# cmavro/GNN-RAG

Measured on AMD Instinct MI355X. Metric: kg_edges_aggregated_per_sec, higher is better.
Workload: dtype f32

## Files before the change

gnn-rag_amd/csrc/dense_internal.h:

```cpp
#pragma once
#include "gnnrag_common.h"

namespace gnnrag {

int tables_vq_launch_z(const gnnrag_csr* csr, const void* planes, const float* ins, const float* W, float* P, int32_t D,
                       int32_t I, int32_t only_dir, float* zero, int64_t zero_n, hipStream_t stream);

int tables_vq_lite_launch_z(const gnnrag_csr* csr, const void* planes, const float* ins, const float* W, float* P, int32_t D,
                            int32_t I, int32_t only_dir, float* zero, int64_t zero_n, hipStream_t stream);

int update_b3_launch_z(const float* h, const float* nbr, const float* W, const float* b, const float* w_s,
                       const float* b_s, const float* mask, float* h_out, float* score, int64_t BN, int32_t D,
                       int32_t ldw, hipStream_t stream, bool score_zeroed);

int update_score_fused_rows(const float* h, const float* nbr, const uint8_t* add_flag, const float* W, const float* b,
                            const float* w_s, const float* b_s, const float* mask, float* h_out, float* score,
                            int64_t BN, int32_t D, int32_t I, int32_t math, hipStream_t stream, bool score_zeroed);
int update_b3_launch_f(const float* h, const float* nbr, const uint8_t* add_flag, const float* W, const float* b,
                       const float* w_s, const float* b_s, const float* mask, float* h_out, float* score, int64_t BN,
                       int32_t D, int32_t ldw, hipStream_t stream, bool score_zeroed);

bool update_rows_supported(const float* h, const float* nbr, const float* W, const float* h_out, int64_t BN, int32_t D,
                           int32_t I, int32_t math);
bool update_b3_shape_ok(int64_t BN, int32_t D, int32_t ldw);
int tables_small_launch(const gnnrag_csr* csr, const float* T_fwd, const float* T_inv, const float* ins, const float* W,
                        float* P, int32_t D, int32_t I, hipStream_t stream);

int frontier_build_z(const gnnrag_csr* csr, const float* dist, void* fws, size_t fws_bytes, float* zero_a,
                     int64_t zero_na, float* zero_b, int64_t zero_nb, hipStream_t stream);
const uint8_t* frontier_row_flags(const gnnrag_csr* csr, const void* fws);

int update_score_fused_z(const float* h, const float* nbr, const float* W, const float* b, const float* w_s,
                         const float* b_s, const float* mask, float* h_out, float* score, int64_t BN, int32_t D,
                         int32_t I, int32_t math, hipStream_t stream, bool score_zeroed);

bool rel_transform_accepts(const float* relfeat_fwd, const float* relfeat_inv, int64_t R1, int32_t D, int32_t L,
                           const gnnrag_layer_params* layers, int32_t pos_rows, const float* T_out, const void* planes_out);

}
```

gnn-rag_amd/csrc/softmax_layer.hip:

```cpp
#include "gnnrag_common.h"
#include "dense_internal.h"

#include <map>
#include <vector>

#ifndef GNNRAG_OVERLAP_TABLES_DEFAULT
#define GNNRAG_OVERLAP_TABLES_DEFAULT 0
#endif
#ifndef GNNRAG_OVERLAP_PROJ_DEFAULT
#define GNNRAG_OVERLAP_PROJ_DEFAULT 0
#endif

namespace gnnrag {

template <int ITEMS>
__global__ __launch_bounds__(1024) void k_masked_softmax(const float* __restrict__ score,
                                                         float* __restrict__ dist, int N) {
  __shared__ float red[16];
  __shared__ float bcast;
  const float* s = score + (size_t)blockIdx.x * N;
  float* o = dist + (size_t)blockIdx.x * N;
  const int lane = threadIdx.x & 63, wave = threadIdx.x >> 6;
  float v[ITEMS > 0 ? ITEMS : 1];

// ... 291 lines not shown
  path &= 0xf;
  if (path == GNNRAG_PATH_AUTO)
    path = fused_is_cheaper(csr->B, csr->N, csr->rel_total, D, I) ? GNNRAG_PATH_FUSED : GNNRAG_PATH_UNFUSED;
  if (path == GNNRAG_PATH_FUSED) {
    float* P = P_done ? P_done : (float*)(base + w.P);
    float* nbr = (float*)(base + w.nbr);
    const bool one_dir = only >= 0 && gnnrag_aggregate_fused_variant(csr, D) != GNNRAG_WALK_L2_GATHER;
    const bool fr_aligned = ((((uintptr_t)ins | (uintptr_t)W_e2e | (uintptr_t)T_fwd | (uintptr_t)T_inv | (uintptr_t)P |
                               (uintptr_t)nbr | (uintptr_t)dist) & 15) == 0) && csr->N > 0;
    const bool frontier_form = seed_prior && only < 0 && fr_aligned && gnnrag_frontier_supported(csr, D) && csr->rel_total > 0;
    if (t_ready && !frontier_form) GNNRAG_HIP(hipStreamWaitEvent((hipStream_t)stream, t_ready, 0));
    if (frontier_form) {
      void* fws = base + w.fws;
      const bool gated = update_rows_supported(h, nbr, W_e2e, h_out, BN, D, I, math);
      if (!gated) GNNRAG_HIP(hipMemsetAsync(nbr, 0, (size_t)BN * D * sizeof(float), (hipStream_t)stream));
      rc = frontier_build_z(csr, dist, fws, w.fws_bytes, score_out, BN, nbr + (size_t)BN * D, D, (hipStream_t)stream);
      if (t_ready) GNNRAG_HIP(hipStreamWaitEvent((hipStream_t)stream, t_ready, 0));
      if (rc) return rc;
      rc = gnnrag_relation_tables_frontier(csr, fws, T_fwd, T_inv, ins, W_e2e, P, D, I, stream);
      if (rc) return rc;
      rc = gnnrag_aggregate_fused_frontier(csr, fws, dist, P, nbr, D, stream);
      if (rc) return rc;
      rc = update_score_fused_rows(h, nbr, gated ? frontier_row_flags(csr, fws) : nullptr, W_e2e, b_e2e, w_score, b_score,
                                   mask, h_out, score_out, BN, D, I, math, (hipStream_t)stream, true);
      if (rc) return rc;
      return finish_softmax(csr, w, base, score_out, dist_out, D, only < 0, pairs_for_next, stream);
    }
    rc = GNNRAG_E_UNSUPPORTED;
    bool score_zeroed = false;
    if (P_done) {
      rc = 0;
      score_zeroed = true;
    } else if (planes && math != GNNRAG_MATH_FP32 && csr->rel_total > 0) {
      const char* menv = getenv("GNNRAG_TABLES_LITE_MAIN");
      rc = ((menv && menv[0] == '1') ? tables_vq_lite_launch_z : tables_vq_launch_z)(
          csr, planes, ins, W_e2e, P, D, I, one_dir ? only : -1, score_out, BN, (hipStream_t)stream);
      score_zeroed = rc == 0;
    }
    if (rc == GNNRAG_E_UNSUPPORTED) rc = gnnrag_relation_tables(csr, T_fwd, T_inv, ins, W_e2e, P, D, I, math, stream);
    if (rc) return rc;
    rc = aggregate_fused_dirs(csr, dist, P, nbr, D, one_dir ? 2 - only : 0, base + w.partial, w.partial_bytes,
                              (hipStream_t)stream, pairs_ready && !one_dir);
    if (rc) return rc;
    rc = update_score_fused_z(h, nbr, W_e2e, b_e2e, w_score, b_score, mask, h_out, score_out, BN, D, I, math,
                              (hipStream_t)stream, score_zeroed);
    if (rc) return rc;
    return finish_softmax(csr, w, base, score_out, dist_out, D, only < 0, pairs_for_next, stream);
  } else {
    if (t_ready) GNNRAG_HIP(hipStreamWaitEvent((hipStream_t)stream, t_ready, 0));
    float* agg = (float*)(base + w.agg);
    rc = gnnrag_aggregate(csr, dist, ins, T_fwd, T_inv, agg, D, I, base + w.partial, w.partial_bytes, stream);
    if (rc) return rc;
    rc = gnnrag_update_score(h, agg, W_e2e, b_e2e, w_score, b_score, mask, h_out, score_out, BN, D, I, math,
                             stream);
    if (rc) return rc;
  }
  return gnnrag_masked_softmax(score_out, dist_out, csr->B, csr->N, stream);
}

static int rel_projections(const gnnrag_csr* csr, int32_t n, const gnnrag_layer_params* layers,
                           const float* relfeat_fwd, const float* relfeat_inv, int32_t pos_rows, float* T,
                           void* planes, bool* planes_written, int32_t D, int32_t math, gnnrag_stream_t stream) {
  *planes_written = false;
  if ((D & 3) == 0) {
    const int rc = gnnrag_rel_transform(relfeat_fwd, relfeat_inv, csr->R1, D, n, layers, pos_rows, T, planes, stream);
    if (rc == 0) *planes_written = planes != nullptr;
    if (rc != GNNRAG_E_UNSUPPORTED) return rc;
  }
// ... 76 lines not shown
  path &= ~GNNRAG_PATH_REUSE_PROJ;
  if (reuse) {
    planes_written = want_planes && rel_transform_accepts(relfeat_fwd, relfeat_inv, csr->R1, D, L, layers, pos_rows, Tall,
                                                          planes_all);
  } else if (upfront) {
    const char* penv = getenv("GNNRAG_OVERLAP_PROJ");
    const bool proj_side = fused && (path & GNNRAG_PATH_SEED_PRIOR) && (penv ? penv[0] != '0' : GNNRAG_OVERLAP_PROJ_DEFAULT != 0);
    OverlapRes* pr = nullptr;
    if (proj_side) {
      const int rc0 = overlap_res(L, &pr);
      if (rc0) return rc0;
      GNNRAG_HIP(hipEventRecord(pr->fork, (hipStream_t)stream));
      GNNRAG_HIP(hipStreamWaitEvent(pr->side, pr->fork, 0));
    }
    const int rc = rel_projections(csr, L, layers, relfeat_fwd, relfeat_inv, pos_rows, Tall,
                                   want_planes ? planes_all : nullptr, &planes_written, D, math,
                                   proj_side ? (gnnrag_stream_t)pr->side : stream);
    if (proj_side) {
      GNNRAG_HIP(hipEventRecord(pr->done[0], pr->side));
      if (rc) (void)hipStreamWaitEvent((hipStream_t)stream, pr->done[0], 0);
      else t_ready = pr->done[0];
    }
    if (rc) return rc;
  }
  const bool overlap = upfront && want_planes && planes_written && fused && (path & ~0xf & ~GNNRAG_PATH_SEED_PRIOR) == 0 &&
                       overlap_shape_ok(csr, L, D, I) && overlap_enabled() &&
                       ((((uintptr_t)ins | (uintptr_t)planes_all) & 15) == 0);
  OverlapRes* ov = nullptr;
  char* P_extra = planes_all + align_up(tables_vq_shape_ok(D, I) ? (size_t)L * plane_bytes : 0, 256);
  const size_t p_bytes = overlap_p_bytes(csr, D);
  bool side_ok[64] = {false};
  const char* genv = getenv("GNNRAG_OVERLAP_GATE");
  const bool gate = !(genv && genv[0] == '0');
  const char* lenv = getenv("GNNRAG_TABLES_LITE");
  const bool lite = !(lenv && lenv[0] == '0');
  auto side_tables = [&](int j) -> int {
    if (j >= 64 || (((uintptr_t)layers[j].W_e2e) & 15) != 0) return 0;
    const int rc = (lite ? tables_vq_lite_launch_z : tables_vq_launch_z)(
        csr, planes_all + (size_t)j * plane_bytes, ins, layers[j].W_e2e, (float*)(P_extra + (size_t)(j - 1) * p_bytes), D, I, -1,
        score_out + (size_t)j * BN, (int64_t)BN, ov->side);
    if (rc == GNNRAG_E_UNSUPPORTED) return 0;
    if (rc) return rc;
    side_ok[j] = true;
    GNNRAG_HIP(hipEventRecord(ov->done[j], ov->side));
    return 0;
  };
  auto side_join_all = [&](int from) {
    if (!ov) return;
    (void)hipEventRecord(ov->done[0], ov->side);
    (void)hipStreamWaitEvent((hipStream_t)stream, ov->done[0], 0);
    (void)from;
  };
  if (overlap && L <= 64) {
    { const int rc = overlap_res(L, &ov); if (rc) return rc; }
    GNNRAG_HIP(hipEventRecord(ov->fork, (hipStream_t)stream));
    GNNRAG_HIP(hipStreamWaitEvent(ov->side, ov->fork, 0));
    int rc_side = 0;
    for (int j = 1; j < (gate ? 2 : L) && !rc_side; ++j) rc_side = side_tables(j);
    if (rc_side) {
      side_join_all(0);
      return rc_side;
    }
  }
  const float* h = h0;
  const float* dist = dist0;
  bool pairs_ready = false;
  for (int j = 0; j < L; ++j) {
    const gnnrag_layer_params& p = layers[j];
    float* hj = h_out + (size_t)j * BN * D;
    float* sj = score_out + (size_t)j * BN;
    float* dj = dist_out + (size_t)j * BN;
// ... 105 lines not shown
```

gnn-rag_amd/csrc/tables_b3.hip:

```cpp
#include "gnnrag_common.h"
#include "dense_internal.h"

namespace gnnrag {

#ifndef GNNRAG_TAB_TPW
#define GNNRAG_TAB_TPW 3
#endif
#ifndef GNNRAG_TAB_MINBLK
#define GNNRAG_TAB_MINBLK 2
#endif
constexpr int kTabTPW = GNNRAG_TAB_TPW;
constexpr int kTabNTH = 7;
constexpr int kTabNKB = 7;
constexpr int kTabSlots = 26;
constexpr int kTabQBytes = 160 * 1024 - 3 * kTabNTH * 16 * kTabSlots * 16 - 64;

struct TabArgs {
  const float* T[2];
  const float* ins;
  const float* W;
  float* P;
  const int2* rows;
  int32_t M, D, I, ldw;
  int32_t ct0;
// ... 204 lines not shown
          }
        }
      }
    }
  }
}

__global__ __launch_bounds__(512, GNNRAG_TAB_MINBLK) void k_tables_b3(TabArgs a) {
  extern __shared__ __attribute__((aligned(16))) unsigned char lds[];
  const int NT = (a.D + 15) >> 4;
  const int h = blockIdx.z;
  const int ctn = h == 0 ? a.ct0 : NT - a.ct0;
  const int col0 = h == 0 ? 0 : a.ct0 * 16;
  const long long U = ((long long)a.M + 15) >> 4;
  const int c0 = (int)(U * blockIdx.x / gridDim.x), c1 = (int)(U * (blockIdx.x + 1) / gridDim.x);
  const int rlo = min(c0 * 16, a.M - 1), rhi = min(c1 * 16, a.M) - 1;
  const int bmin = a.rows[rlo].x, bmax = a.rows[max(rhi, rlo)].x;
  const int nq = bmax - bmin + 1;
  const bool q_in_lds = (size_t)nq * a.I * a.D * sizeof(float) <= kTabQBytes;
#define GNNRAG_TAB_CASE(N)                                                  \
  case N:                                                                   \
    if (q_in_lds) tables_b3_part<N, true>(a, lds, col0, bmin, nq);          \
    else tables_b3_part<N, false>(a, lds, col0, bmin, nq);                  \
    break;
  switch (ctn) {
    GNNRAG_TAB_CASE(6) GNNRAG_TAB_CASE(7)
    default: break;
  }
#undef GNNRAG_TAB_CASE
}

constexpr int kVqHalf = 32 * kTabNKB;
constexpr int kVqRowB = 2 * kVqHalf * 2;
#ifndef GNNRAG_VQ_TPW
#define GNNRAG_VQ_TPW 5
#endif
#ifndef GNNRAG_VQ_UN
#define GNNRAG_VQ_UN 3
#endif
constexpr int kVqTPW = GNNRAG_VQ_TPW;

struct VqArgs {
  const unsigned char* planes;
  const float* ins;
  const float* W;
  float* P;
  const int2* rows;
  const int* rel_off;
  int32_t M, D, I, ldw, R1;
  int32_t ct0;
  int32_t nchunk;
  int32_t dir0;
  float* zero;
  int64_t zero_n;
};

template <int CTN, int UN>
__device__ __forceinline__ void vq_stage(const VqArgs& a, unsigned char* lds, const float* qarea, int col0, int ncol,
                                         int d, int s) {
  constexpr int RB = kTabSlots * 16;
  constexpr int PL = kTabNTH * 16 * RB;
  const int tid = threadIdx.x;
  const int D = a.D, I = a.I, KC = D >> 2;
  const f32x4 zero4 = {0.f, 0.f, 0.f, 0.f};
  const int total = tab_stage_rows(CTN) * kTabSlots * 2;
  for (int base = 0; base < total; base += 512 * UN) {
    f32x4 v[UN];
#pragma unroll
    for (int u = 0; u < UN; ++u) v[u] = zero4;
    for (int i = 0; i < I; ++i) {
      f32x4 w[UN];
      const float* wsrc = a.W + (size_t)col0 * a.ldw + (1 + 2 * i + d) * D;
#pragma unroll
      for (int u = 0; u < UN; ++u) {
        const int idx = base + u * 512 + tid;
        const int j = idx / (kTabSlots * 2), kc = idx - j * (kTabSlots * 2);
        w[u] = *reinterpret_cast<const f32x4*>(wsrc + (size_t)min(j, ncol - 1) * a.ldw + 4 * min(kc, KC - 1));
      }
#pragma unroll
      for (int u = 0; u < UN; ++u) {
        const int idx = base + u * 512 + tid;
        const int kc = idx % (kTabSlots * 2);
        f32x4 q = *reinterpret_cast<const f32x4*>(qarea + i * D + 4 * min(kc, KC - 1));
        q = __builtin_elementwise_max(s ? -q : q, zero4);
        v[u] += w[u] * q;
      }
    }
#pragma unroll
    for (int u = 0; u < UN; ++u) {
      const int idx = base + u * 512 + tid;
      const int j = idx / (kTabSlots * 2), kc = idx - j * (kTabSlots * 2);
      if (idx < total) {
        const Split3 sp = split3(j < ncol && kc < KC ? v[u] : zero4);
        unsigned char* dst = lds + tab_lds_row(j) * RB + kc * 8;
        *reinterpret_cast<uint2*>(dst) = sp.hi;
        *reinterpret_cast<uint2*>(dst + PL) = sp.mid;
        *reinterpret_cast<uint2*>(dst + 2 * PL) = sp.lo;
      }
    }
  }
}

template <int CTN>
__device__ __forceinline__ void tables_vq_part(const VqArgs& a, unsigned char* lds, int col0) {
  constexpr int RB = kTabSlots * 16;
  constexpr int PL = kTabNTH * 16 * RB;
  constexpr int NKB = kTabNKB;
  const int tid = threadIdx.x, lane = tid & 63, wave = tid >> 6;
  const int fr = lane & 15, fg = lane >> 4;
  const int d = a.dir0 + blockIdx.y;
  const int g = blockIdx.x / a.nchunk, ch = blockIdx.x - g * a.nchunk;
  const int D = a.D, I = a.I;
  const int r0 = a.rel_off[g], r1 = a.rel_off[g + 1];
  if (r1 <= r0) return;
  const int ncol = min(CTN * 16, D - col0);
  const int KC = D >> 2;
  const f32x4 zero4 = {0.f, 0.f, 0.f, 0.f};
  float* P = a.P + (size_t)d * a.M * D;
  const unsigned char* planes = a.planes + (size_t)d * 3 * a.R1 * kVqRowB;
  const size_t plane_stride = (size_t)a.R1 * kVqRowB;

  const int U = (r1 - r0 + 15) >> 4;
  const int c0 = U * ch / a.nchunk, c1 = U * (ch + 1) / a.nchunk;
  const int wv = __builtin_amdgcn_readfirstlane(wave);
  const int w0 = c0 + (c1 - c0) * wv / 8, w1 = c0 + (c1 - c0) * (wv + 1) / 8;
  const int npass = ((c1 - c0 + 7) / 8 + kVqTPW - 1) / kVqTPW;

  if (tid < 16) reinterpret_cast<unsigned*>(lds + 3 * PL)[tid] = 0u;
  float* qarea = reinterpret_cast<float*>(lds + 3 * PL + 64);
  for (int x = tid * 4; x < I * D; x += 512 * 4)
    *reinterpret_cast<f32x4*>(qarea + x) = *reinterpret_cast<const f32x4*>(a.ins + (size_t)g * I * D + x);

  for (int pass = 0; pass < npass; ++pass) {
    const int tbase = w0 + pass * kVqTPW;
    const int ntile = max(0, min(kVqTPW, w1 - tbase));
    f32x4 acc[kVqTPW][CTN];
#pragma unroll
    for (int j = 0; j < kVqTPW; ++j)
#pragma unroll
      for (int nt = 0; nt < CTN; ++nt) acc[j][nt] = zero4;
    unsigned aoff[kVqTPW];
#pragma unroll
    for (int j = 0; j < kVqTPW; ++j) {
      const int m = min(r0 + (tbase + (j < ntile ? j : 0)) * 16 + fr, r1 - 1);
      aoff[j] = (unsigned)a.rows[m].y * (unsigned)kVqRowB + (unsigned)fg * 16u;
    }
    const unsigned char* const plane_base[3] = {planes, planes + plane_stride, planes + 2 * plane_stride};

    for (int s = 0; s < 2; ++s) {
      __syncthreads();
      vq_stage<CTN, GNNRAG_VQ_UN>(a, lds, qarea, col0, ncol, d, s);
      __syncthreads();

      bf16x8 ap[kVqTPW][3];
#pragma unroll
      for (int j = 0; j < kVqTPW; ++j)
#pragma unroll
        for (int pl = 0; pl < 3; ++pl)
          ap[j][pl] = __builtin_bit_cast(bf16x8, *reinterpret_cast<const f32x4*>(plane_base[pl] + (aoff[j] + (unsigned)(s * (kVqHalf * 2)))));
      for (int kb = 0; kb < NKB; ++kb) {
        const int kbn = min(kb + 1, NKB - 1);
        const unsigned char* wb = lds + fr * RB + kb * 64 + fg * 16;
        constexpr int PA[6] = {1, 2, 0, 1, 0, 0};
        constexpr int PB[6] = {1, 0, 2, 0, 1, 0};
#pragma unroll
        for (int j = 0; j < kVqTPW; ++j) {
          if (j < ntile) {
#pragma unroll
            for (int nt = 0; nt < CTN; nt += 2) {
              bf16x8 b0[3], b1[3];
#pragma unroll
              for (int pl = 0; pl < 3; ++pl) {
                b0[pl] = __builtin_bit_cast(bf16x8, *reinterpret_cast<const f32x4*>(wb + pl * PL + nt * 16 * RB));
                b1[pl] = b0[pl];
                if (nt + 1 < CTN)
                  b1[pl] = __builtin_bit_cast(bf16x8, *reinterpret_cast<const f32x4*>(wb + pl * PL + (nt + 1) * 16 * RB));
              }
#pragma unroll
              for (int p = 0; p < 6; ++p) {
                acc[j][nt] = __builtin_amdgcn_mfma_f32_16x16x32_bf16(ap[j][PA[p]], b0[PB[p]], acc[j][nt], 0, 0, 0);
                if (nt + 1 < CTN)
                  acc[j][nt + 1] = __builtin_amdgcn_mfma_f32_16x16x32_bf16(ap[j][PA[p]], b1[PB[p]], acc[j][nt + 1], 0, 0, 0);
              }
            }
          }
#pragma unroll
          for (int pl = 0; pl < 3; ++pl)
            ap[j][pl] = __builtin_bit_cast(bf16x8, *reinterpret_cast<const f32x4*>(plane_base[pl] + (aoff[j] + (unsigned)(s * (kVqHalf * 2) + kbn * 64))));
        }
      }
    }

#pragma unroll
    for (int j = 0; j < kVqTPW; ++j) {
      if (j < ntile) {
        const int rbase = r0 + (tbase + j) * 16 + 4 * fg;
#pragma unroll
        for (int q = 0; q < 4; ++q) {
          const int row = rbase + q;
          if (row < r1) {
            float* prow = P + (size_t)row * D + col0;
            static_assert(CTN >= 4, "a column part holds at least the interleaved group");
            {
              const f32x4 v = {acc[j][0][q], acc[j][1][q], acc[j][2][q], acc[j][3][q]};
              const int c = 4 * fr;
              if (c + 4 <= ncol) *reinterpret_cast<f32x4*>(prow + c) = v;
              else {
#pragma unroll
                for (int e = 0; e < 4; ++e)
                  if (c + e < ncol) prow[c + e] = v[e];
              }
            }
#pragma unroll
            for (int nt = 4; nt < CTN; ++nt) {
              const int c = nt * 16 + fr;
              if (c < ncol) prow[c] = acc[j][nt][q];
            }
          }
        }
      }
    }
  }
}

__global__ __launch_bounds__(512, 2) void k_tables_vq(VqArgs a) {
  extern __shared__ __attribute__((aligned(16))) unsigned char lds[];
  if (a.zero) {
    const int64_t nb = (int64_t)gridDim.x * gridDim.y * gridDim.z;
    const int64_t lin = blockIdx.x + (int64_t)gridDim.x * (blockIdx.y + (int64_t)gridDim.y * blockIdx.z);
    for (int64_t i = lin * 512 + threadIdx.x; i < a.zero_n; i += nb * 512) a.zero[i] = 0.f;
  }
  const int NT = (a.D + 15) >> 4;
  const int h = blockIdx.z;
  const int ctn = h == 0 ? a.ct0 : NT - a.ct0;
  const int col0 = h == 0 ? 0 : a.ct0 * 16;
  switch (ctn) {
    case 6: tables_vq_part<6>(a, lds, col0); break;
    case 7: tables_vq_part<7>(a, lds, col0); break;
    default: break;
  }
}

constexpr int kVlThreads = 256;
constexpr int kVlWaves = kVlThreads / 64;
#ifndef GNNRAG_VL_TPW
#define GNNRAG_VL_TPW 10
#endif
constexpr int kVlTPW = GNNRAG_VL_TPW;
constexpr int kVlCT = 3;
#ifndef GNNRAG_VL_NB
#define GNNRAG_VL_NB 5
#endif
constexpr int kVlNB = GNNRAG_VL_NB;
static_assert(kVlTPW % kVlNB == 0, "the A-fragment ring keeps its phase from one k block to the next");

__device__ __forceinline__ int vl_lds_row(int j, int ctn) { return ctn >= 4 ? tab_lds_row(j) : j; }

template <int CTN, int UN>
__device__ __forceinline__ void vl_stage(const VqArgs& a, unsigned char* lds, const float* qarea, int col0, int ncol,
                                         int d, int s) {
  constexpr int RB = kTabSlots * 16;
  constexpr int PL = kVlCT * 16 * RB;
  const int tid = threadIdx.x;
  const int D = a.D, I = a.I, KC = D >> 2;
  const f32x4 zero4 = {0.f, 0.f, 0.f, 0.f};
  constexpr int rows = CTN < kVlCT ? CTN * 16 + 1 : CTN * 16;
  const int total = rows * kTabSlots * 2;
  for (int base = 0; base < total; base += kVlThreads * UN) {
    f32x4 v[UN];
#pragma unroll
    for (int u = 0; u < UN; ++u) v[u] = zero4;
    for (int i = 0; i < I; ++i) {
      f32x4 w[UN];
      const float* wsrc = a.W + (size_t)col0 * a.ldw + (1 + 2 * i + d) * D;
#pragma unroll
      for (int u = 0; u < UN; ++u) {
        const int idx = base + u * kVlThreads + tid;
        const int j = idx / (kTabSlots * 2), kc = idx - j * (kTabSlots * 2);
        w[u] = *reinterpret_cast<const f32x4*>(wsrc + (size_t)min(j, ncol - 1) * a.ldw + 4 * min(kc, KC - 1));
      }
#pragma unroll
      for (int u = 0; u < UN; ++u) {
        const int idx = base + u * kVlThreads + tid;
        const int kc = idx % (kTabSlots * 2);
        f32x4 q = *reinterpret_cast<const f32x4*>(qarea + i * D + 4 * min(kc, KC - 1));
        q = __builtin_elementwise_max(s ? -q : q, zero4);
        v[u] += w[u] * q;
      }
    }
#pragma unroll
    for (int u = 0; u < UN; ++u) {
      const int idx = base + u * kVlThreads + tid;
      const int j = idx / (kTabSlots * 2), kc = idx - j * (kTabSlots * 2);
      if (idx < total) {
        const Split3 sp = split3(j < ncol && kc < KC ? v[u] : zero4);
        unsigned char* dst = lds + vl_lds_row(j, CTN) * RB + kc * 8;
        *reinterpret_cast<uint2*>(dst) = sp.hi;
        *reinterpret_cast<uint2*>(dst + PL) = sp.mid;
        *reinterpret_cast<uint2*>(dst + 2 * PL) = sp.lo;
      }
    }
  }
}

template <int CTN>
__device__ __forceinline__ void tables_vl_part(const VqArgs& a, unsigned char* lds, int col0) {
  constexpr int RB = kTabSlots * 16;
  constexpr int PL = kVlCT * 16 * RB;
  constexpr int NKB = kTabNKB;
  constexpr int TPW = kVlTPW;
  const int tid = threadIdx.x, lane = tid & 63, wave = tid >> 6;
  const int fr = lane & 15, fg = lane >> 4;
  const int d = a.dir0 + blockIdx.y;
  const int g = blockIdx.x / a.nchunk, ch = blockIdx.x - g * a.nchunk;
  const int D = a.D, I = a.I;
  const int r0 = a.rel_off[g], r1 = a.rel_off[g + 1];
  if (r1 <= r0) return;
  const int ncol = min(CTN * 16, D - col0);
  const f32x4 zero4 = {0.f, 0.f, 0.f, 0.f};
  float* P = a.P + (size_t)d * a.M * D;
  const unsigned char* planes = a.planes + (size_t)d * 3 * a.R1 * kVqRowB;
  const size_t plane_stride = (size_t)a.R1 * kVqRowB;

  const int U = (r1 - r0 + 15) >> 4;
  const int c0 = U * ch / a.nchunk, c1 = U * (ch + 1) / a.nchunk;
  const int wv = __builtin_amdgcn_readfirstlane(wave);
  const int w0 = c0 + (c1 - c0) * wv / kVlWaves, w1 = c0 + (c1 - c0) * (wv + 1) / kVlWaves;
  const int npass = ((c1 - c0 + kVlWaves - 1) / kVlWaves + TPW - 1) / TPW;

  if (tid < 16) reinterpret_cast<unsigned*>(lds + 3 * PL)[tid] = 0u;
  float* qarea = reinterpret_cast<float*>(lds + 3 * PL + 64);
  for (int x = tid * 4; x < I * D; x += kVlThreads * 4)
    *reinterpret_cast<f32x4*>(qarea + x) = *reinterpret_cast<const f32x4*>(a.ins + (size_t)g * I * D + x);

  for (int pass = 0; pass < npass; ++pass) {
    const int tbase = w0 + pass * TPW;
    const int ntile = max(0, min(TPW, w1 - tbase));
    f32x4 acc[TPW][CTN];
#pragma unroll
    for (int j = 0; j < TPW; ++j)
#pragma unroll
      for (int nt = 0; nt < CTN; ++nt) acc[j][nt] = zero4;
    unsigned aoff[TPW];
#pragma unroll
    for (int j = 0; j < TPW; ++j) {
      const int m = min(r0 + (tbase + (j < ntile ? j : 0)) * 16 + fr, r1 - 1);
      aoff[j] = (unsigned)a.rows[m].y * (unsigned)kVqRowB + (unsigned)fg * 16u;
    }
    const unsigned char* const plane_base[3] = {planes, planes + plane_stride, planes + 2 * plane_stride};

    for (int s = 0; s < 2; ++s) {
      __syncthreads();
      vl_stage<CTN, 3>(a, lds, qarea, col0, ncol, d, s);
      __syncthreads();

      constexpr int NB = kVlNB;
      bf16x8 ap[NB][3];
#pragma unroll
      for (int j = 0; j < NB - 1; ++j)
#pragma unroll
        for (int pl = 0; pl < 3; ++pl)
          ap[j][pl] = __builtin_bit_cast(bf16x8, *reinterpret_cast<const f32x4*>(plane_base[pl] + (aoff[j] + (unsigned)(s * (kVqHalf * 2)))));
      for (int kb = 0; kb < NKB; ++kb) {
        const int kbn = min(kb + 1, NKB - 1);
        const unsigned char* wb = lds + fr * RB + kb * 64 + fg * 16;
        constexpr int PA[6] = {1, 2, 0, 1, 0, 0};
        constexpr int PB[6] = {1, 0, 2, 0, 1, 0};
        bf16x8 bfr[CTN][3];
#pragma unroll
        for (int nt = 0; nt < CTN; ++nt)
#pragma unroll
          for (int pl = 0; pl < 3; ++pl)
            bfr[nt][pl] = __builtin_bit_cast(bf16x8, *reinterpret_cast<const f32x4*>(wb + pl * PL + nt * 16 * RB));
#pragma unroll
        for (int j = 0; j < TPW; ++j) {
          {
            constexpr int AH = NB - 1;
            const unsigned nxt = j + AH < TPW ? aoff[j + AH < TPW ? j + AH : 0] + (unsigned)(s * (kVqHalf * 2) + kb * 64)
                                              : aoff[j + AH < TPW ? 0 : j + AH - TPW] + (unsigned)(s * (kVqHalf * 2) + kbn * 64);
#pragma unroll
            for (int pl = 0; pl < 3; ++pl)
              ap[(j + AH) % NB][pl] = __builtin_bit_cast(bf16x8, *reinterpret_cast<const f32x4*>(plane_base[pl] + nxt));
          }
          if (j < ntile) {
#pragma unroll
            for (int p = 0; p < 6; ++p)
#pragma unroll
              for (int nt = 0; nt < CTN; ++nt)
                acc[j][nt] = __builtin_amdgcn_mfma_f32_16x16x32_bf16(ap[j % NB][PA[p]], bfr[nt][PB[p]], acc[j][nt], 0, 0, 0);
          }
          __builtin_amdgcn_sched_barrier(0);
        }
      }
    }

#pragma unroll
    for (int j = 0; j < TPW; ++j) {
      if (j < ntile) {
        const int rbase = r0 + (tbase + j) * 16 + 4 * fg;
#pragma unroll
        for (int q = 0; q < 4; ++q) {
          const int row = rbase + q;
          if (row < r1) {
            float* prow = P + (size_t)row * D + col0;
            if constexpr (CTN >= 4) {
              const f32x4 v = {acc[j][0][q], acc[j][1][q], acc[j][2][q], acc[j][3][q]};
              const int c = 4 * fr;
              if (c + 4 <= ncol) *reinterpret_cast<f32x4*>(prow + c) = v;
              else {
#pragma unroll
                for (int e = 0; e < 4; ++e)
                  if (c + e < ncol) prow[c + e] = v[e];
              }
            } else {
#pragma unroll
              for (int nt = 0; nt < CTN; ++nt) {
                const int c = nt * 16 + fr;
                if (c < ncol) prow[c] = acc[j][nt][q];
              }
            }
          }
        }
      }
    }
  }
}

__global__ __launch_bounds__(kVlThreads, 2) void k_tables_vq_lite(VqArgs a) {
  extern __shared__ __attribute__((aligned(16))) unsigned char lds[];
  if (a.zero) {
    const int64_t nb = (int64_t)gridDim.x * gridDim.y * gridDim.z;
    const int64_t lin = blockIdx.x + (int64_t)gridDim.x * (blockIdx.y + (int64_t)gridDim.y * blockIdx.z);
    for (int64_t i = lin * kVlThreads + threadIdx.x; i < a.zero_n; i += nb * kVlThreads) a.zero[i] = 0.f;
  }
  const int h = blockIdx.z;
  if (h < 3) tables_vl_part<3>(a, lds, h * 48);
  else tables_vl_part<2>(a, lds, 144 + (h - 3) * 32);
}

struct UpdB3Args {
  const float* A;
  const float* W;
  const float* bias;
  const float* add;
  const float* w_s;
  const float* b_s;
  const float* mask;
  float* C;
  float* score;
  const uint8_t* add_flag;
  int32_t M, D, ldw, ct0;
};

template <int CTN, bool FL>
__device__ __forceinline__ void update_b3_part(const UpdB3Args& a, unsigned char* lds, int col0, bool first_part,
                                               int chunk, int nchunks) {
  constexpr int RB = kTabSlots * 16;
  constexpr int PL = kTabNTH * 16 * RB;
  constexpr int NKB = kTabNKB;
  const int tid = threadIdx.x, lane = tid & 63, wave = tid >> 6;
  const int fr = lane & 15, fg = lane >> 4;
  const int D = a.D;
  const int ncol = min(CTN * 16, D - col0);
  const int KC = D >> 2;
  const f32x4 zero4 = {0.f, 0.f, 0.f, 0.f};
  float* Bl = reinterpret_cast<float*>(lds + 3 * PL + 64);
  float* Sl = Bl + kTabNTH * 16;

  if (tid < 16) reinterpret_cast<unsigned*>(lds + 3 * PL)[tid] = 0u;
  for (int j = tid; j < kTabNTH * 16; j += 512) {
// ... 240 lines not shown
  if (!tables_vq_shape_ok(D, I) || csr->rel_total < 1024 || only_dir > 1) return GNNRAG_E_UNSUPPORTED;
  if ((((uintptr_t)planes | (uintptr_t)ins | (uintptr_t)W | (uintptr_t)P) & 15) != 0) return GNNRAG_E_UNSUPPORTED;
  VqArgs a;
  memset(&a, 0, sizeof(a));
  a.planes = (const unsigned char*)planes; a.ins = ins; a.W = W; a.P = P;
  a.rows = (const int2*)csr->rel_rows; a.rel_off = csr->rel_off;
  a.M = csr->rel_total; a.D = D; a.I = I; a.ldw = (2 * I + 1) * D; a.R1 = csr->R1;
  const int NT = (D + 15) / 16;
  a.ct0 = (NT + 1) / 2;
  int cus = 0;
  {
    const int rc = device_cu_count(&cus);
    if (rc) return rc;
  }
  const int ndir = only_dir < 0 ? 2 : 1;
  a.dir0 = only_dir < 0 ? 0 : only_dir;
  int nchunk = cus / (csr->B * 2 * ndir);
  const int tiles_max = (csr->rel_max + 15) / 16;
  if (nchunk > tiles_max / 8) nchunk = tiles_max / 8;
  if (nchunk < 1) nchunk = 1;
  a.nchunk = nchunk;
  a.zero = zero;
  a.zero_n = zero ? zero_n : 0;
  static DeviceMask cap;
  {
    const int rc = raise_lds_cap(k_tables_vq, cap);
    if (rc) return rc;
  }
  hipLaunchKernelGGL(k_tables_vq, dim3(csr->B * nchunk, ndir, 2), dim3(512), 160 * 1024, stream, a);
  GNNRAG_LAUNCH_CHECK();
  return 0;
}

int tables_vq_lite_launch_z(const gnnrag_csr* csr, const void* planes, const float* ins, const float* W, float* P, int32_t D,
                            int32_t I, int32_t only_dir, float* zero, int64_t zero_n, hipStream_t stream) {
  if (!tables_vq_shape_ok(D, I) || csr->rel_total < 1024 || only_dir > 1) return GNNRAG_E_UNSUPPORTED;
  if ((((uintptr_t)planes | (uintptr_t)ins | (uintptr_t)W | (uintptr_t)P) & 15) != 0) return GNNRAG_E_UNSUPPORTED;
  VqArgs a;
  memset(&a, 0, sizeof(a));
  a.planes = (const unsigned char*)planes; a.ins = ins; a.W = W; a.P = P;
  a.rows = (const int2*)csr->rel_rows; a.rel_off = csr->rel_off;
  a.M = csr->rel_total; a.D = D; a.I = I; a.ldw = (2 * I + 1) * D; a.R1 = csr->R1;
  a.ct0 = kVlCT;
  int cus = 0;
  {
    const int rc = device_cu_count(&cus);
    if (rc) return rc;
  }
  const int ndir = only_dir < 0 ? 2 : 1;
  a.dir0 = only_dir < 0 ? 0 : only_dir;
  int nchunk = cus / (csr->B * 5 * ndir);
  const int tiles_max = (csr->rel_max + 15) / 16;
  if (nchunk > tiles_max / 8) nchunk = tiles_max / 8;
  if (nchunk < 1) nchunk = 1;
  a.nchunk = nchunk;
  a.zero = zero;
  a.zero_n = zero ? zero_n : 0;
  static DeviceMask cap;
  {
    const int rc = raise_lds_cap(k_tables_vq_lite, cap);
    if (rc) return rc;
  }
  size_t lds = (size_t)3 * kVlCT * 16 * kTabSlots * 16 + 64 + (size_t)I * D * sizeof(float);
  if (const char* e = getenv("GNNRAG_VL_LDS_KB")) {
    const size_t want = (size_t)atoi(e) * 1024;
    if (want > lds && want <= 160 * 1024) lds = want;
  }
  hipLaunchKernelGGL(k_tables_vq_lite, dim3(csr->B * nchunk, ndir, 5), dim3(kVlThreads), lds, stream, a);
  GNNRAG_LAUNCH_CHECK();
  return 0;
}

int tables_b3_launch(const gnnrag_csr* csr, const float* T_fwd, const float* T_inv, const float* ins, const float* W,
                     float* P, int32_t D, int32_t I, hipStream_t stream) {
  if (D % 8 || (D + 31) / 32 != kTabNKB || (D + 15) / 16 != 13 || csr->rel_total < 1024) return GNNRAG_E_UNSUPPORTED;
  if ((((uintptr_t)T_fwd | (uintptr_t)T_inv | (uintptr_t)ins | (uintptr_t)W | (uintptr_t)P) & 15) != 0)
    return GNNRAG_E_UNSUPPORTED;
  TabArgs a;
  memset(&a, 0, sizeof(a));
  a.T[0] = T_fwd; a.T[1] = T_inv; a.ins = ins; a.W = W; a.P = P;
  a.rows = (const int2*)csr->rel_rows;
  a.M = csr->rel_total; a.D = D; a.I = I; a.ldw = (2 * I + 1) * D;
  const int NT = (D + 15) / 16;
  a.ct0 = NT <= kTabNTH ? NT : (NT + 1) / 2;
  const int parts = NT <= kTabNTH ? 1 : 2;
  int cus = 0;
  {
    const int rc = device_cu_count(&cus);
    if (rc) return rc;
  }
  const long long U = ((long long)a.M + 15) / 16;
  int chunks = cus / (2 * parts);
  if (chunks < 1) chunks = 1;
  if ((long long)chunks * 8 > U) chunks = (int)((U + 7) / 8);
  const int tiles_per_wave = (int)((((U + chunks - 1) / chunks) + 7) / 8);
  a.npass = (tiles_per_wave + kTabTPW - 1) / kTabTPW;
  const size_t lds = 160 * 1024;
  static DeviceMask cap;
  {
    const int rc = raise_lds_cap(k_tables_b3, cap);
    if (rc) return rc;
  }
  hipLaunchKernelGGL(k_tables_b3, dim3(chunks, 2, parts), dim3(512), lds, stream, a);
  GNNRAG_LAUNCH_CHECK();
  return 0;
// ... 11 lines not shown
```

Before: 2.995 billion.

## Merge sign halves into sparse MFMA and drop lite tables kernel

The relation-table kernel used to run two passes, one for the positive and one for the negative relu half of the query. It now stages both halves interleaved into LDS per k-block group and feeds them to structured-sparse smfmac 16x16x64 instructions. A sparsity index is derived from the plane bits, which assumes that in each pair only one of the two entries is nonzero. The separate lite tables kernel and its env switches are removed, so the overlap side path now uses the main kernel instead of lite, which was its default. Staging unroll drops from 3 to 2, and staging now happens in k-block chunks, which adds more syncs.

```diff
diff --git a/gnn-rag_amd/csrc/dense_internal.h b/gnn-rag_amd/csrc/dense_internal.h
--- a/gnn-rag_amd/csrc/dense_internal.h
+++ b/gnn-rag_amd/csrc/dense_internal.h
@@ -5,9 +5,6 @@
 
 int tables_vq_launch_z(const gnnrag_csr* csr, const void* planes, const float* ins, const float* W, float* P, int32_t D,
                        int32_t I, int32_t only_dir, float* zero, int64_t zero_n, hipStream_t stream);
-
-int tables_vq_lite_launch_z(const gnnrag_csr* csr, const void* planes, const float* ins, const float* W, float* P, int32_t D,
-                            int32_t I, int32_t only_dir, float* zero, int64_t zero_n, hipStream_t stream);
 
 int update_b3_launch_z(const float* h, const float* nbr, const float* W, const float* b, const float* w_s,
                        const float* b_s, const float* mask, float* h_out, float* score, int64_t BN, int32_t D,
diff --git a/gnn-rag_amd/csrc/softmax_layer.hip b/gnn-rag_amd/csrc/softmax_layer.hip
--- a/gnn-rag_amd/csrc/softmax_layer.hip
+++ b/gnn-rag_amd/csrc/softmax_layer.hip
@@ -347,8 +347,7 @@
       rc = 0;
       score_zeroed = true;
     } else if (planes && math != GNNRAG_MATH_FP32 && csr->rel_total > 0) {
-      const char* menv = getenv("GNNRAG_TABLES_LITE_MAIN");
-      rc = ((menv && menv[0] == '1') ? tables_vq_lite_launch_z : tables_vq_launch_z)(
+      rc = tables_vq_launch_z(
           csr, planes, ins, W_e2e, P, D, I, one_dir ? only : -1, score_out, BN, (hipStream_t)stream);
       score_zeroed = rc == 0;
     }
@@ -491,11 +490,9 @@
   bool side_ok[64] = {false};
   const char* genv = getenv("GNNRAG_OVERLAP_GATE");
   const bool gate = !(genv && genv[0] == '0');
-  const char* lenv = getenv("GNNRAG_TABLES_LITE");
-  const bool lite = !(lenv && lenv[0] == '0');
   auto side_tables = [&](int j) -> int {
     if (j >= 64 || (((uintptr_t)layers[j].W_e2e) & 15) != 0) return 0;
-    const int rc = (lite ? tables_vq_lite_launch_z : tables_vq_launch_z)(
+    const int rc = tables_vq_launch_z(
         csr, planes_all + (size_t)j * plane_bytes, ins, layers[j].W_e2e, (float*)(P_extra + (size_t)(j - 1) * p_bytes), D, I, -1,
         score_out + (size_t)j * BN, (int64_t)BN, ov->side);
     if (rc == GNNRAG_E_UNSUPPORTED) return 0;
diff --git a/gnn-rag_amd/csrc/tables_b3.hip b/gnn-rag_amd/csrc/tables_b3.hip
--- a/gnn-rag_amd/csrc/tables_b3.hip
+++ b/gnn-rag_amd/csrc/tables_b3.hip
@@ -260,11 +260,13 @@
 
 constexpr int kVqHalf = 32 * kTabNKB;
 constexpr int kVqRowB = 2 * kVqHalf * 2;
+constexpr int kVqStageKB = 3;
+static_assert(kVqStageKB * 128 < kTabSlots * 16, "a stage's k blocks fit an LDS plane row");
 #ifndef GNNRAG_VQ_TPW
 #define GNNRAG_VQ_TPW 5
 #endif
 #ifndef GNNRAG_VQ_UN
-#define GNNRAG_VQ_UN 3
+#define GNNRAG_VQ_UN 2
 #endif
 constexpr int kVqTPW = GNNRAG_VQ_TPW;
 
@@ -283,47 +285,72 @@
   int64_t zero_n;
 };
 
-template <int CTN, int UN>
+typedef __bf16 bf16x16 __attribute__((ext_vector_type(16)));
+__device__ __forceinline__ bf16x16 lds_bf16x16(const unsigned char* p) {
+  const uint4 lo = *reinterpret_cast<const uint4*>(p), hi = *reinterpret_cast<const uint4*>(p + 64);
+  typedef unsigned u32x8 __attribute__((ext_vector_type(8)));
+  const u32x8 v = {lo.x, lo.y, lo.z, lo.w, hi.x, hi.y, hi.z, hi.w};
+  return __builtin_bit_cast(bf16x16, v);
+}
+
+__device__ __forceinline__ int vq_pair_index(uint4 m) {
+  const unsigned f0 = ((m.x & 0x7fff7fffu) + 0x7fff7fffu) & 0x80008000u;
+  const unsigned f1 = ((m.y & 0x7fff7fffu) + 0x7fff7fffu) & 0x80008000u;
+  const unsigned f2 = ((m.z & 0x7fff7fffu) + 0x7fff7fffu) & 0x80008000u;
+  const unsigned f3 = ((m.w & 0x7fff7fffu) + 0x7fff7fffu) & 0x80008000u;
+  const unsigned g = (f0 >> 15) | (f1 >> 11) | (f2 >> 7) | (f3 >> 3);
+  return (int)(0x8888u | (g & 0x1111u) | ((g >> 14) & 0x4444u));
+}
+
+__device__ __forceinline__ uint2 vq_interleave(unsigned p, unsigned m) {
+  return make_uint2((p & 0xffffu) | (m << 16), (p >> 16) | (m & 0xffff0000u));
+}
+
+template <int CTN, int UN, int NKS>
 __device__ __forceinline__ void vq_stage(const VqArgs& a, unsigned char* lds, const float* qarea, int col0, int ncol,
-                                         int d, int s) {
+                                         int d, int kb0) {
   constexpr int RB = kTabSlots * 16;
   constexpr int PL = kTabNTH * 16 * RB;
   const int tid = threadIdx.x;
   const int D = a.D, I = a.I, KC = D >> 2;
   const f32x4 zero4 = {0.f, 0.f, 0.f, 0.f};
-  const int total = tab_stage_rows(CTN) * kTabSlots * 2;
+  constexpr int total = CTN * 16 * NKS * 8;
   for (int base = 0; base < total; base += 512 * UN) {
-    f32x4 v[UN];
-#pragma unroll
-    for (int u = 0; u < UN; ++u) v[u] = zero4;
+    f32x4 vp[UN], vm[UN];
+#pragma unroll
+    for (int u = 0; u < UN; ++u) vp[u] = vm[u] = zero4;
     for (int i = 0; i < I; ++i) {
       f32x4 w[UN];
       const float* wsrc = a.W + (size_t)col0 * a.ldw + (1 + 2 * i + d) * D;
 #pragma unroll
       for (int u = 0; u < UN; ++u) {
         const int idx = base + u * 512 + tid;
-        const int j = idx / (kTabSlots * 2), kc = idx - j * (kTabSlots * 2);
+        const int j = idx / (NKS * 8), kc = kb0 * 8 + (idx - j * (NKS * 8));
         w[u] = *reinterpret_cast<const f32x4*>(wsrc + (size_t)min(j, ncol - 1) * a.ldw + 4 * min(kc, KC - 1));
       }
 #pragma unroll
       for (int u = 0; u < UN; ++u) {
         const int idx = base + u * 512 + tid;
-        const int kc = idx % (kTabSlots * 2);
-        f32x4 q = *reinterpret_cast<const f32x4*>(qarea + i * D + 4 * min(kc, KC - 1));
-        q = __builtin_elementwise_max(s ? -q : q, zero4);
-        v[u] += w[u] * q;
+        const int kc = kb0 * 8 + idx % (NKS * 8);
+        const f32x4 q = *reinterpret_cast<const f32x4*>(qarea + i * D + 4 * min(kc, KC - 1));
+        vp[u] += w[u] * __builtin_elementwise_max(q, zero4);
+        vm[u] += w[u] * __builtin_elementwise_max(-q, zero4);
       }
     }
 #pragma unroll
     for (int u = 0; u < UN; ++u) {
       const int idx = base + u * 512 + tid;
-      const int j = idx / (kTabSlots * 2), kc = idx - j * (kTabSlots * 2);
+      const int j = idx / (NKS * 8), r = idx - j * (NKS * 8), kc = kb0 * 8 + r;
       if (idx < total) {
-        const Split3 sp = split3(j < ncol && kc < KC ? v[u] : zero4);
-        unsigned char* dst = lds + tab_lds_row(j) * RB + kc * 8;
-        *reinterpret_cast<uint2*>(dst) = sp.hi;
-        *reinterpret_cast<uint2*>(dst + PL) = sp.mid;
-        *reinterpret_cast<uint2*>(dst + 2 * PL) = sp.lo;
+        const bool live = j < ncol && kc < KC;
+        const Split3 sp = split3(live ? vp[u] : zero4), sm = split3(live ? vm[u] : zero4);
+        unsigned char* dst = lds + tab_lds_row(j) * RB + (r >> 3) * 128 + (r & 7) * 16;
+        const uint2 h0 = vq_interleave(sp.hi.x, sm.hi.x), h1 = vq_interleave(sp.hi.y, sm.hi.y);
+        const uint2 m0 = vq_interleave(sp.mid.x, sm.mid.x), m1 = vq_interleave(sp.mid.y, sm.mid.y);
+        const uint2 l0 = vq_interleave(sp.lo.x, sm.lo.x), l1 = vq_interleave(sp.lo.y, sm.lo.y);
+        *reinterpret_cast<uint4*>(dst) = make_uint4(h0.x, h0.y, h1.x, h1.y);
+        *reinterpret_cast<uint4*>(dst + PL) = make_uint4(m0.x, m0.y, m1.x, m1.y);
+        *reinterpret_cast<uint4*>(dst + 2 * PL) = make_uint4(l0.x, l0.y, l1.x, l1.y);
       }
     }
   }
@@ -342,7 +369,6 @@
   const int r0 = a.rel_off[g], r1 = a.rel_off[g + 1];
   if (r1 <= r0) return;
   const int ncol = min(CTN * 16, D - col0);
-  const int KC = D >> 2;
   const f32x4 zero4 = {0.f, 0.f, 0.f, 0.f};
   float* P = a.P + (size_t)d * a.M * D;
   const unsigned char* planes = a.planes + (size_t)d * 3 * a.R1 * kVqRowB;
@@ -354,7 +380,6 @@
   const int w0 = c0 + (c1 - c0) * wv / 8, w1 = c0 + (c1 - c0) * (wv + 1) / 8;
   const int npass = ((c1 - c0 + 7) / 8 + kVqTPW - 1) / kVqTPW;
 
-  if (tid < 16) reinterpret_cast<unsigned*>(lds + 3 * PL)[tid] = 0u;
   float* qarea = reinterpret_cast<float*>(lds + 3 * PL + 64);
   for (int x = tid * 4; x < I * D; x += 512 * 4)
     *reinterpret_cast<f32x4*>(qarea + x) = *reinterpret_cast<const f32x4*>(a.ins + (size_t)g * I * D + x);
@@ -375,46 +400,51 @@
     }
     const unsigned char* const plane_base[3] = {planes, planes + plane_stride, planes + 2 * plane_stride};
 
-    for (int s = 0; s < 2; ++s) {
+    uint4 rp[3], rm[3];
+#pragma unroll
+    for (int pl = 0; pl < 3; ++pl) {
+      rp[pl] = *reinterpret_cast<const uint4*>(plane_base[pl] + aoff[0]);
+      rm[pl] = *reinterpret_cast<const uint4*>(plane_base[pl] + (aoff[0] + (unsigned)(kVqHalf * 2)));
+    }
+
+    for (int kb0 = 0; kb0 < NKB; kb0 += kVqStageKB) {
       __syncthreads();
-      vq_stage<CTN, GNNRAG_VQ_UN>(a, lds, qarea, col0, ncol, d, s);
+      if (kb0 + kVqStageKB <= NKB) vq_stage<CTN, GNNRAG_VQ_UN, kVqStageKB>(a, lds, qarea, col0, ncol, d, kb0);
+      else vq_stage<CTN, GNNRAG_VQ_UN, NKB % kVqStageKB>(a, lds, qarea, col0, ncol, d, kb0);
       __syncthreads();
 
-      bf16x8 ap[kVqTPW][3];
-#pragma unroll
-      for (int j = 0; j < kVqTPW; ++j)
-#pragma unroll
-        for (int pl = 0; pl < 3; ++pl)
-          ap[j][pl] = __builtin_bit_cast(bf16x8, *reinterpret_cast<const f32x4*>(plane_base[pl] + (aoff[j] + (unsigned)(s * (kVqHalf * 2)))));
-      for (int kb = 0; kb < NKB; ++kb) {
+      const int kb1 = min(kb0 + kVqStageKB, NKB);
+      for (int kb = kb0; kb < kb1; ++kb) {
         const int kbn = min(kb + 1, NKB - 1);
-        const unsigned char* wb = lds + fr * RB + kb * 64 + fg * 16;
+        const unsigned char* wb = lds + fr * RB + (kb - kb0) * 128 + fg * 16;
         constexpr int PA[6] = {1, 2, 0, 1, 0, 0};
         constexpr int PB[6] = {1, 0, 2, 0, 1, 0};
 #pragma unroll
         for (int j = 0; j < kVqTPW; ++j) {
           if (j < ntile) {
-#pragma unroll
-            for (int nt = 0; nt < CTN; nt += 2) {
-              bf16x8 b0[3], b1[3];
+            bf16x8 ap[3];
+#pragma unroll
+            for (int pl = 0; pl < 3; ++pl) ap[pl] = __builtin_bit_cast(bf16x8, rp[pl] | rm[pl]);
+            const int sidx = vq_pair_index(rm[0]);
+            {
+              const unsigned nxt = j + 1 < ntile ? aoff[j + 1 < kVqTPW ? j + 1 : 0] + (unsigned)(kb * 64)
+                                                 : aoff[0] + (unsigned)(kbn * 64);
 #pragma unroll
               for (int pl = 0; pl < 3; ++pl) {
-                b0[pl] = __builtin_bit_cast(bf16x8, *reinterpret_cast<const f32x4*>(wb + pl * PL + nt * 16 * RB));
-                b1[pl] = b0[pl];
-                if (nt + 1 < CTN)
-                  b1[pl] = __builtin_bit_cast(bf16x8, *reinterpret_cast<const f32x4*>(wb + pl * PL + (nt + 1) * 16 * RB));
+                rp[pl] = *reinterpret_cast<const uint4*>(plane_base[pl] + nxt);
+                rm[pl] = *reinterpret_cast<const uint4*>(plane_base[pl] + (nxt + (unsigned)(kVqHalf * 2)));
               }
-#pragma unroll
-              for (int p = 0; p < 6; ++p) {
-                acc[j][nt] = __builtin_amdgcn_mfma_f32_16x16x32_bf16(ap[j][PA[p]], b0[PB[p]], acc[j][nt], 0, 0, 0);
-                if (nt + 1 < CTN)
-                  acc[j][nt + 1] = __builtin_amdgcn_mfma_f32_16x16x32_bf16(ap[j][PA[p]], b1[PB[p]], acc[j][nt + 1], 0, 0, 0);
-              }
+            }
+#pragma unroll
+            for (int nt = 0; nt < CTN; ++nt) {
+              bf16x16 b[3];
+#pragma unroll
+              for (int pl = 0; pl < 3; ++pl) b[pl] = lds_bf16x16(wb + pl * PL + nt * 16 * RB);
+#pragma unroll
+              for (int p = 0; p < 6; ++p)
+                acc[j][nt] = __builtin_amdgcn_smfmac_f32_16x16x64_bf16(ap[PA[p]], b[PB[p]], acc[j][nt], sidx, 0, 0);
             }
           }
-#pragma unroll
-          for (int pl = 0; pl < 3; ++pl)
-            ap[j][pl] = __builtin_bit_cast(bf16x8, *reinterpret_cast<const f32x4*>(plane_base[pl] + (aoff[j] + (unsigned)(s * (kVqHalf * 2) + kbn * 64))));
         }
       }
     }
@@ -467,203 +497,6 @@
     case 7: tables_vq_part<7>(a, lds, col0); break;
     default: break;
   }
-}
-
-constexpr int kVlThreads = 256;
-constexpr int kVlWaves = kVlThreads / 64;
-#ifndef GNNRAG_VL_TPW
-#define GNNRAG_VL_TPW 10
-#endif
-constexpr int kVlTPW = GNNRAG_VL_TPW;
-constexpr int kVlCT = 3;
-#ifndef GNNRAG_VL_NB
-#define GNNRAG_VL_NB 5
-#endif
-constexpr int kVlNB = GNNRAG_VL_NB;
-static_assert(kVlTPW % kVlNB == 0, "the A-fragment ring keeps its phase from one k block to the next");
-
-__device__ __forceinline__ int vl_lds_row(int j, int ctn) { return ctn >= 4 ? tab_lds_row(j) : j; }
-
-template <int CTN, int UN>
-__device__ __forceinline__ void vl_stage(const VqArgs& a, unsigned char* lds, const float* qarea, int col0, int ncol,
-                                         int d, int s) {
-  constexpr int RB = kTabSlots * 16;
-  constexpr int PL = kVlCT * 16 * RB;
-  const int tid = threadIdx.x;
-  const int D = a.D, I = a.I, KC = D >> 2;
-  const f32x4 zero4 = {0.f, 0.f, 0.f, 0.f};
-  constexpr int rows = CTN < kVlCT ? CTN * 16 + 1 : CTN * 16;
-  const int total = rows * kTabSlots * 2;
-  for (int base = 0; base < total; base += kVlThreads * UN) {
-    f32x4 v[UN];
-#pragma unroll
-    for (int u = 0; u < UN; ++u) v[u] = zero4;
-    for (int i = 0; i < I; ++i) {
-      f32x4 w[UN];
-      const float* wsrc = a.W + (size_t)col0 * a.ldw + (1 + 2 * i + d) * D;
-#pragma unroll
-      for (int u = 0; u < UN; ++u) {
-        const int idx = base + u * kVlThreads + tid;
-        const int j = idx / (kTabSlots * 2), kc = idx - j * (kTabSlots * 2);
-        w[u] = *reinterpret_cast<const f32x4*>(wsrc + (size_t)min(j, ncol - 1) * a.ldw + 4 * min(kc, KC - 1));
-      }
-#pragma unroll
-      for (int u = 0; u < UN; ++u) {
-        const int idx = base + u * kVlThreads + tid;
-        const int kc = idx % (kTabSlots * 2);
-        f32x4 q = *reinterpret_cast<const f32x4*>(qarea + i * D + 4 * min(kc, KC - 1));
-        q = __builtin_elementwise_max(s ? -q : q, zero4);
-        v[u] += w[u] * q;
-      }
-    }
-#pragma unroll
-    for (int u = 0; u < UN; ++u) {
-      const int idx = base + u * kVlThreads + tid;
-      const int j = idx / (kTabSlots * 2), kc = idx - j * (kTabSlots * 2);
-      if (idx < total) {
-        const Split3 sp = split3(j < ncol && kc < KC ? v[u] : zero4);
-        unsigned char* dst = lds + vl_lds_row(j, CTN) * RB + kc * 8;
-        *reinterpret_cast<uint2*>(dst) = sp.hi;
-        *reinterpret_cast<uint2*>(dst + PL) = sp.mid;
-        *reinterpret_cast<uint2*>(dst + 2 * PL) = sp.lo;
-      }
-    }
-  }
-}
-
-template <int CTN>
-__device__ __forceinline__ void tables_vl_part(const VqArgs& a, unsigned char* lds, int col0) {
-  constexpr int RB = kTabSlots * 16;
-  constexpr int PL = kVlCT * 16 * RB;
-  constexpr int NKB = kTabNKB;
-  constexpr int TPW = kVlTPW;
-  const int tid = threadIdx.x, lane = tid & 63, wave = tid >> 6;
-  const int fr = lane & 15, fg = lane >> 4;
-  const int d = a.dir0 + blockIdx.y;
-  const int g = blockIdx.x / a.nchunk, ch = blockIdx.x - g * a.nchunk;
-  const int D = a.D, I = a.I;
-  const int r0 = a.rel_off[g], r1 = a.rel_off[g + 1];
-  if (r1 <= r0) return;
-  const int ncol = min(CTN * 16, D - col0);
-  const f32x4 zero4 = {0.f, 0.f, 0.f, 0.f};
-  float* P = a.P + (size_t)d * a.M * D;
-  const unsigned char* planes = a.planes + (size_t)d * 3 * a.R1 * kVqRowB;
-  const size_t plane_stride = (size_t)a.R1 * kVqRowB;
-
-  const int U = (r1 - r0 + 15) >> 4;
-  const int c0 = U * ch / a.nchunk, c1 = U * (ch + 1) / a.nchunk;
-  const int wv = __builtin_amdgcn_readfirstlane(wave);
-  const int w0 = c0 + (c1 - c0) * wv / kVlWaves, w1 = c0 + (c1 - c0) * (wv + 1) / kVlWaves;
-  const int npass = ((c1 - c0 + kVlWaves - 1) / kVlWaves + TPW - 1) / TPW;
-
-  if (tid < 16) reinterpret_cast<unsigned*>(lds + 3 * PL)[tid] = 0u;
-  float* qarea = reinterpret_cast<float*>(lds + 3 * PL + 64);
-  for (int x = tid * 4; x < I * D; x += kVlThreads * 4)
-    *reinterpret_cast<f32x4*>(qarea + x) = *reinterpret_cast<const f32x4*>(a.ins + (size_t)g * I * D + x);
-
-  for (int pass = 0; pass < npass; ++pass) {
-    const int tbase = w0 + pass * TPW;
-    const int ntile = max(0, min(TPW, w1 - tbase));
-    f32x4 acc[TPW][CTN];
-#pragma unroll
-    for (int j = 0; j < TPW; ++j)
-#pragma unroll
-      for (int nt = 0; nt < CTN; ++nt) acc[j][nt] = zero4;
-    unsigned aoff[TPW];
-#pragma unroll
-    for (int j = 0; j < TPW; ++j) {
-      const int m = min(r0 + (tbase + (j < ntile ? j : 0)) * 16 + fr, r1 - 1);
-      aoff[j] = (unsigned)a.rows[m].y * (unsigned)kVqRowB + (unsigned)fg * 16u;
-    }
-    const unsigned char* const plane_base[3] = {planes, planes + plane_stride, planes + 2 * plane_stride};
-
-    for (int s = 0; s < 2; ++s) {
-      __syncthreads();
-      vl_stage<CTN, 3>(a, lds, qarea, col0, ncol, d, s);
-      __syncthreads();
-
-      constexpr int NB = kVlNB;
-      bf16x8 ap[NB][3];
-#pragma unroll
-      for (int j = 0; j < NB - 1; ++j)
-#pragma unroll
-        for (int pl = 0; pl < 3; ++pl)
-          ap[j][pl] = __builtin_bit_cast(bf16x8, *reinterpret_cast<const f32x4*>(plane_base[pl] + (aoff[j] + (unsigned)(s * (kVqHalf * 2)))));
-      for (int kb = 0; kb < NKB; ++kb) {
-        const int kbn = min(kb + 1, NKB - 1);
-        const unsigned char* wb = lds + fr * RB + kb * 64 + fg * 16;
-        constexpr int PA[6] = {1, 2, 0, 1, 0, 0};
-        constexpr int PB[6] = {1, 0, 2, 0, 1, 0};
-        bf16x8 bfr[CTN][3];
-#pragma unroll
-        for (int nt = 0; nt < CTN; ++nt)
-#pragma unroll
-          for (int pl = 0; pl < 3; ++pl)
-            bfr[nt][pl] = __builtin_bit_cast(bf16x8, *reinterpret_cast<const f32x4*>(wb + pl * PL + nt * 16 * RB));
-#pragma unroll
-        for (int j = 0; j < TPW; ++j) {
-          {
-            constexpr int AH = NB - 1;
-            const unsigned nxt = j + AH < TPW ? aoff[j + AH < TPW ? j + AH : 0] + (unsigned)(s * (kVqHalf * 2) + kb * 64)
-                                              : aoff[j + AH < TPW ? 0 : j + AH - TPW] + (unsigned)(s * (kVqHalf * 2) + kbn * 64);
-#pragma unroll
-            for (int pl = 0; pl < 3; ++pl)
-              ap[(j + AH) % NB][pl] = __builtin_bit_cast(bf16x8, *reinterpret_cast<const f32x4*>(plane_base[pl] + nxt));
-          }
-          if (j < ntile) {
-#pragma unroll
-            for (int p = 0; p < 6; ++p)
-#pragma unroll
-              for (int nt = 0; nt < CTN; ++nt)
-                acc[j][nt] = __builtin_amdgcn_mfma_f32_16x16x32_bf16(ap[j % NB][PA[p]], bfr[nt][PB[p]], acc[j][nt], 0, 0, 0);
-          }
-          __builtin_amdgcn_sched_barrier(0);
-        }
-      }
-    }
-
-#pragma unroll
-    for (int j = 0; j < TPW; ++j) {
-      if (j < ntile) {
-        const int rbase = r0 + (tbase + j) * 16 + 4 * fg;
-#pragma unroll
-        for (int q = 0; q < 4; ++q) {
-          const int row = rbase + q;
-          if (row < r1) {
-            float* prow = P + (size_t)row * D + col0;
-            if constexpr (CTN >= 4) {
-              const f32x4 v = {acc[j][0][q], acc[j][1][q], acc[j][2][q], acc[j][3][q]};
-              const int c = 4 * fr;
-              if (c + 4 <= ncol) *reinterpret_cast<f32x4*>(prow + c) = v;
-              else {
-#pragma unroll
-                for (int e = 0; e < 4; ++e)
-                  if (c + e < ncol) prow[c + e] = v[e];
-              }
-            } else {
-#pragma unroll
-              for (int nt = 0; nt < CTN; ++nt) {
-                const int c = nt * 16 + fr;
-                if (c < ncol) prow[c] = acc[j][nt][q];
-              }
-            }
-          }
-        }
-      }
-    }
-  }
-}
-
-__global__ __launch_bounds__(kVlThreads, 2) void k_tables_vq_lite(VqArgs a) {
-  extern __shared__ __attribute__((aligned(16))) unsigned char lds[];
-  if (a.zero) {
-    const int64_t nb = (int64_t)gridDim.x * gridDim.y * gridDim.z;
-    const int64_t lin = blockIdx.x + (int64_t)gridDim.x * (blockIdx.y + (int64_t)gridDim.y * blockIdx.z);
-    for (int64_t i = lin * kVlThreads + threadIdx.x; i < a.zero_n; i += nb * kVlThreads) a.zero[i] = 0.f;
-  }
-  const int h = blockIdx.z;
-  if (h < 3) tables_vl_part<3>(a, lds, h * 48);
-  else tables_vl_part<2>(a, lds, 144 + (h - 3) * 32);
 }
 
 struct UpdB3Args {
@@ -970,45 +803,6 @@
   return 0;
 }
 
-int tables_vq_lite_launch_z(const gnnrag_csr* csr, const void* planes, const float* ins, const float* W, float* P, int32_t D,
-                            int32_t I, int32_t only_dir, float* zero, int64_t zero_n, hipStream_t stream) {
-  if (!tables_vq_shape_ok(D, I) || csr->rel_total < 1024 || only_dir > 1) return GNNRAG_E_UNSUPPORTED;
-  if ((((uintptr_t)planes | (uintptr_t)ins | (uintptr_t)W | (uintptr_t)P) & 15) != 0) return GNNRAG_E_UNSUPPORTED;
-  VqArgs a;
-  memset(&a, 0, sizeof(a));
-  a.planes = (const unsigned char*)planes; a.ins = ins; a.W = W; a.P = P;
-  a.rows = (const int2*)csr->rel_rows; a.rel_off = csr->rel_off;
-  a.M = csr->rel_total; a.D = D; a.I = I; a.ldw = (2 * I + 1) * D; a.R1 = csr->R1;
-  a.ct0 = kVlCT;
-  int cus = 0;
-  {
-    const int rc = device_cu_count(&cus);
-    if (rc) return rc;
-  }
-  const int ndir = only_dir < 0 ? 2 : 1;
-  a.dir0 = only_dir < 0 ? 0 : only_dir;
-  int nchunk = cus / (csr->B * 5 * ndir);
-  const int tiles_max = (csr->rel_max + 15) / 16;
-  if (nchunk > tiles_max / 8) nchunk = tiles_max / 8;
-  if (nchunk < 1) nchunk = 1;
-  a.nchunk = nchunk;
-  a.zero = zero;
-  a.zero_n = zero ? zero_n : 0;
-  static DeviceMask cap;
-  {
-    const int rc = raise_lds_cap(k_tables_vq_lite, cap);
-    if (rc) return rc;
-  }
-  size_t lds = (size_t)3 * kVlCT * 16 * kTabSlots * 16 + 64 + (size_t)I * D * sizeof(float);
-  if (const char* e = getenv("GNNRAG_VL_LDS_KB")) {
-    const size_t want = (size_t)atoi(e) * 1024;
-    if (want > lds && want <= 160 * 1024) lds = want;
-  }
-  hipLaunchKernelGGL(k_tables_vq_lite, dim3(csr->B * nchunk, ndir, 5), dim3(kVlThreads), lds, stream, a);
-  GNNRAG_LAUNCH_CHECK();
-  return 0;
-}
-
 int tables_b3_launch(const gnnrag_csr* csr, const float* T_fwd, const float* T_inv, const float* ins, const float* W,
                      float* P, int32_t D, int32_t I, hipStream_t stream) {
   if (D % 8 || (D + 31) / 32 != kTabNKB || (D + 15) / 16 != 13 || csr->rel_total < 1024) return GNNRAG_E_UNSUPPORTED;
```

After: 3.033 billion (median of 6 runs). 1.01x the previous value.
